# TinfoilHat0/Defending-Against-Backdoors-with-Robust-Learning-Rate

Measured on NVIDIA H100. Metric: fl_rounds_per_sec, higher is better.
Workload: dtype bf16

## Files before the change

### defending-against-backdoors-with-robust-learning-rate_b200/models/native.py

```python
from __future__ import annotations

import math
import os

import torch
import torch.nn.functional as F

from .. import ops
from .graph import FlatLayout

ACT = torch.bfloat16
FUSE_DROPOUT = bool(int(os.environ.get("RLR_FUSE_DROPOUT", "1")))
FUSE_RELU_POOL = bool(int(os.environ.get("RLR_FUSE_RELU_POOL", "1")))
EPILOGUE_BN_STATS = bool(int(os.environ.get("RLR_EPILOGUE_BN_STATS", "0")))
FWD_BRANCH = bool(int(os.environ.get("RLR_FWD_BRANCH", "1")))
BWD_BRANCH = bool(int(os.environ.get("RLR_BWD_BRANCH", "1")))
EPI_STAT_SLOTS = min(16, max(1, int(os.environ.get("RLR_EPI_STAT_SLOTS", "2"))))
FWD_SLOTS = BWD_SLOTS = max(1, int(os.environ.get("RLR_BN_SLOTS", "1")))
WGRAD_OVERLAP = bool(int(os.environ.get("RLR_WGRAD_OVERLAP", "1")))


def dropout_stream_base(seed: int, agent_id: int, rnd: int) -> int:
    z = (int(seed) * 0x9E3779B97F4A7C15 + (int(agent_id) + 1) * 0xBF58476D1CE4E5B9 + (int(rnd) + 1) * 0x94D049BB133111EB) & (2 ** 64 - 1)
    z = ((z ^ (z >> 30)) * 0xBF58476D1CE4E5B9) & (2 ** 64 - 1)
# ... 348 lines not shown
        name = op.name + ".weight"
        gw, gb = self.pg[name], self.pg.get(op.name + ".bias")
        s, p = a.get("stride", 1), a.get("pad", 0)
        if self.impl["conv_wgrad"] == "sm100" and ops.conv_supported(op.in_shape, a, "wgrad"):
            if getattr(self, "_side", None) is not None:
                self._side.wait_stream(torch.cuda.current_stream(self.device))
                with torch.cuda.stream(self._side):
                    ops.conv2d_wgrad_sm100(x, dy, gw, gb, s, p, tag=(id(self), op.name), zero=False)
            else:
                ops.conv2d_wgrad_sm100(x, dy, gw, gb, s, p, tag=(id(self), op.name), zero=False)
        else:
            if self.impl["conv_wgrad"] == "sm100":
                ops.note_fallback("conv_wgrad", f"{op.name} in={op.in_shape} {a}")
            _, dw, db = torch.ops.aten.convolution_backward(
                dy.permute(0, 3, 1, 2), x.permute(0, 3, 1, 2), self.pwb[name].permute(0, 3, 1, 2),
                [a["cout"]] if gb is not None else None, [s, s], [p, p], [1, 1], False, [0, 0], 1, [False, True, gb is not None])
            gw.copy_(dw.permute(0, 2, 3, 1))
            if gb is not None:
                gb.copy_(db)
        if not op.need_dx:
            return
        dx = self.G(op.x, B)
        if self.impl["conv_dgrad"] == "sm100" and ops.conv_supported(op.in_shape, a, "dgrad"):
            ops.conv2d_dgrad_sm100(dy, self.pwb[name], dx, s, p, op.acc_dx)
            return
        if self.impl["conv_dgrad"] == "sm100":
            ops.note_fallback("conv_dgrad", f"{op.name} in={op.in_shape} {a}")
        di, _, _ = torch.ops.aten.convolution_backward(
            dy.permute(0, 3, 1, 2), x.permute(0, 3, 1, 2), self.pwb[name].permute(0, 3, 1, 2), None, [s, s], [p, p], [1, 1],
            False, [0, 0], 1, [True, False, False])
        di = di.permute(0, 2, 3, 1)
        if op.acc_dx:
            dx.add_(di)
        else:
            dx.copy_(di)

    def _fwd_bn(self, op, B, train):
        a = op.attrs
        x, y = self.T(op.x, B), self.T(op.y, B)
        res = self.T(op.res, B) if op.res is not None else None
        gamma, beta = self.pw[op.name + ".weight"], self.pw[op.name + ".bias"]
        rm, rv = self.pw[op.name + ".running_mean"], self.pw[op.name + ".running_var"]
        prod = op.saved["producer"]
        stats = prod.saved["stats"] if (train and prod is not None and prod.saved.get("stats_done")) else None
        if stats is not None and not self.fuse_bn_stats:
            stats = stats[0:EPI_STAT_SLOTS]
        count = x.numel() // x.shape[-1]
# ... 230 lines not shown
```

### defending-against-backdoors-with-robust-learning-rate_b200/ops/__init__.py

```python
from __future__ import annotations

import importlib.util
import os
import threading
from typing import NamedTuple

import numpy as np
import torch

_HERE = os.path.dirname(os.path.abspath(__file__))
_SO = os.path.join(_HERE, "_C.so")
_ext = None
_ext_err = None
_lock = threading.Lock()

MODE_IDS = {"avg": 0, "comed": 1, "sign": 2}
MAX_FUSED_AGENTS = 1024


class _Counter:
    calls = 0


class _CountingExt:
# ... 429 lines not shown
        dl = dl.to(logits.dtype)
        if dlogits is not None:
            dlogits.copy_(dl)
            dl = dlogits
    if loss_sum is None:
        loss_sum = torch.zeros(1)
    loss_sum += loss
    if correct is not None:
        correct += (lf.argmax(1) == labels).sum().to(correct.dtype)
    return loss_sum, dl


def eval_metrics(logits, labels, loss_sum, confusion):
    if logits.is_cuda:
        ext().eval_metrics(logits.contiguous(), labels, loss_sum, confusion)
        return
    lf = logits.float()
    loss_sum += torch.nn.functional.cross_entropy(lf, labels, reduction="sum").double()
    C = lf.shape[1]
    pred = lf.argmax(1)
    confusion.view(-1).index_add_(0, labels * C + pred, torch.ones_like(labels))


from .nn import (avgpool_bwd, avgpool_fwd, bn_bwd, bn_fwd, conv2d_dgrad_sm100, conv2d_fwd_sm100, conv2d_wgrad_sm100, conv_supported,
                 dropout_bwd, dropout_fwd, gn_bwd, gn_fwd, linear_bwd, linear_fused_dropout_ok, linear_fwd, maxpool2_bwd, maxpool2_fwd, relu_bwd_, scratch, stem_geometry, STAT_SLOTS)
```

### defending-against-backdoors-with-robust-learning-rate_b200/ops/csrc/gemm.cu

```cuda
#include <cuda.h>
#include <stdlib.h>

#include "common.cuh"
#include "gemm.h"
#include "stem_gather.cuh"
#include "wgmma.cuh"

namespace rlr {

using namespace wg;

constexpr int BM = 128;
constexpr int BK = 64;
constexpr int kConsumers = 256;
constexpr int kThreads = kConsumers + 64;
constexpr int kEpiThreads = kConsumers;

template <int BN, int kOcc = 2>
struct TileCfg {
    static constexpr int kStages = kOcc == 3 ? (BN == 64 ? 3 : 2) : (BN == 64 ? 4 : 3);
    static constexpr int kABytes = BM * BK * 2;
    static constexpr int kBBytes = BN * BK * 2;
    static constexpr int kStageBytes = kABytes + kBBytes;
    static constexpr int kPitch = BN * 2 + 16;
// ... 445 lines not shown
cudaError_t launch_stem_gemm_bf16(const void* A, const void* W, void* out, int M, int N, int kvalid, int ldw, const float* bias, int relu,
                                  float* stats, const uint32_t* wait_flags, int wait_lo, int wait_hi, const uint32_t* wait_epoch,
                                  cudaStream_t st) {
    if (N % 8 || M <= 0 || kvalid < 1 || kvalid > BK || ldw < kvalid) return cudaErrorInvalidValue;
    if (wait_flags && (!wait_epoch || wait_lo > wait_hi || wait_lo < 0)) return cudaErrorInvalidValue;
    const int m_tiles = (M + BM - 1) / BM;
    const int bn = pick_bn(N);
    CUtensorMap tmA;
    {
        const uint64_t d[2] = {(uint64_t)BK, (uint64_t)M}, s[1] = {(uint64_t)BK * 2};
        const uint32_t b[2] = {BK, BM};
        RLR_CUDA_CHECK(make_tmap_bf16(&tmA, A, 2, d, s, b));
    }
    ConvGemmParams p{};
    p.M = M; p.N = N; p.num_kb = 1; p.mode = 0; p.in_stride = 1; p.out_stride = 1;
    p.out = out; p.ldc = N; p.bias = bias; p.stats = stats; p.relu = relu; p.accumulate = 0;
    p.b_src = reinterpret_cast<const __nv_bfloat16*>(W); p.b_ld = ldw; p.b_kvalid = kvalid;
    p.wait_flags = wait_flags; p.wait_lo = wait_lo; p.wait_hi = wait_hi; p.wait_epoch = wait_epoch;
    return bn == 128 ? launch_bn<128>(tmA, tmA, p, m_tiles, st) : launch_bn<64>(tmA, tmA, p, m_tiles, st);
}

static int pow2_ceil(int x) { int p = 1; while (p < x) p <<= 1; return p; }

cudaError_t launch_conv_bf16(const void* x, const void* w, void* out, int NB, int planes, int Hin, int Win, int Cin, int Ho, int Wo,
                             int Cout, int ldc, int ntaps, const int* dh, const int* dw, const int* dplane, const float* bias,
                             int relu, int accumulate, float* stats, cudaStream_t st, const int* wtap, int w_taps_total,
                             int in_stride, int out_stride, int out_ph, int out_pw) {
    if (Cin % BK || Cout % 8 || ntaps < 1 || ntaps > 9) return cudaErrorInvalidValue;
    if (in_stride < 1 || in_stride > 2 || out_stride < 1 || out_stride > 2 || (in_stride > 1 && planes != 1)) return cudaErrorInvalidValue;
    if (wtap && (stats || Cout % 64)) return cudaErrorInvalidValue;
    int bn = pick_bn(Cout);
    ConvGemmParams p{};
    {
        static const int small_bn64 = [] { const char* e = getenv("RLR_SMALL_BN64"); return e ? atoi(e) : 1; }();
        const long long px = (long long)NB * Ho * Wo;
        if (small_bn64 && bn == 128 && ((px + BM - 1) / BM) * (Cout / 128) < sm_count()) bn = 64;
    }
    int TW = pow2_ceil(Wo); if (TW > BM) TW = BM;
    int TH = pow2_ceil(Ho); if (TW * TH > BM) TH = BM / TW;
    int TN = BM / (TW * TH);
    p.TW = TW; p.TH = TH; p.TN = TN;
    p.tiles_w = (Wo + TW - 1) / TW; p.tiles_h = (Ho + TH - 1) / TH;
    const int tiles_n = (NB + TN - 1) / TN;
    const int m_tiles = p.tiles_w * p.tiles_h * tiles_n;
    p.M = NB * Ho * Wo; p.N = Cout; p.mode = 1; p.cblocks = Cin / BK; p.num_kb = ntaps * p.cblocks; p.ntaps = ntaps;
    p.Ho = Ho; p.Wo = Wo; p.NB = NB;
    p.in_stride = in_stride; p.out_stride = out_stride; p.out_ph = out_ph; p.out_pw = out_pw; p.OutH = Ho * out_stride; p.OutW = Wo * out_stride;
    for (int t = 0; t < ntaps; ++t) { p.dh[t] = (int8_t)dh[t]; p.dw[t] = (int8_t)dw[t]; p.dn[t] = dplane[t] * NB; }
    p.out = out; p.ldc = ldc; p.bias = bias; p.stats = stats; p.relu = relu; p.accumulate = accumulate;
    CUtensorMap tmA, tmB;
    {
        const uint64_t d[4] = {(uint64_t)Cin, (uint64_t)Win, (uint64_t)Hin, (uint64_t)planes * NB};
        const uint64_t s[3] = {(uint64_t)Cin * 2, (uint64_t)Win * Cin * 2, (uint64_t)Hin * Win * Cin * 2};
        const uint32_t b[4] = {BK, (uint32_t)TW, (uint32_t)TH, (uint32_t)TN};
        const uint32_t es[4] = {1, (uint32_t)in_stride, (uint32_t)in_stride, 1};
        RLR_CUDA_CHECK(make_tmap_bf16(&tmA, x, 4, d, s, b, in_stride > 1 ? es : nullptr));
    }
    if (wtap) {
        if (bias) return cudaErrorInvalidValue;
        p.b_mn = 1; p.wcols = Cout;
        for (int t = 0; t < ntaps; ++t) p.wtap[t] = wtap[t];
        const uint64_t cols = (uint64_t)w_taps_total * Cout;
        const uint64_t d[2] = {cols, (uint64_t)Cin}, s[1] = {cols * 2};
        const uint32_t b[2] = {64, BK};
        RLR_CUDA_CHECK(make_tmap_bf16(&tmB, w, 2, d, s, b));
    } else {
        const uint64_t K = (uint64_t)ntaps * Cin;
        const uint64_t d[2] = {K, (uint64_t)Cout}, s[1] = {K * 2};
        const uint32_t b[2] = {BK, (uint32_t)bn};
        RLR_CUDA_CHECK(make_tmap_bf16(&tmB, w, 2, d, s, b));
    }
    return bn == 128 ? launch_bn<128>(tmA, tmB, p, m_tiles, st) : launch_bn<64>(tmA, tmB, p, m_tiles, st);
}

}
```

### defending-against-backdoors-with-robust-learning-rate_b200/ops/csrc/gemm.h

```cpp
#pragma once
#include <cuda_runtime.h>
#include <cuda_bf16.h>
#include <stdint.h>

#include "dropspec.h"

namespace rlr {

constexpr int kStatSlots = 16;

struct ConvGemmParams {
    int M, N, num_kb;
    int mode;
    int cblocks;
    int TW, TH, TN;
    int Ho, Wo, NB;
    int tiles_w, tiles_h;
    int ntaps;
    int in_stride;
    int out_stride, out_ph, out_pw, OutH, OutW;
    int8_t dh[9], dw[9];
    int dn[9];
    int b_mn;
    int wtap[9];
    int wcols;
    DropSpec drop;
    int tma_store;
    int split_prod;
    long long* dbg;
    const __nv_bfloat16* b_src;
    int b_ld, b_kvalid;
    const uint32_t* wait_flags;
    int wait_lo, wait_hi;
    const uint32_t* wait_epoch;
    void* out;
    int ldc;
    const float* bias;
    float* stats;
    int stat_slots;
    int relu, accumulate;
};

cudaError_t launch_gemm_bf16(const void* A, const void* B, void* out, int M, int N, int K, int lda, int ldb, int ldc,
                             const float* bias, int relu, int accumulate, float* stats, cudaStream_t st, const DropSpec* drop = nullptr);
cudaError_t launch_stem_gemm_bf16(const void* A, const void* W, void* out, int M, int N, int kvalid, int ldw, const float* bias, int relu,
                                  float* stats, const uint32_t* wait_flags, int wait_lo, int wait_hi, const uint32_t* wait_epoch,
                                  cudaStream_t st);
void set_pdl(int on);
cudaError_t launch_gemm_splitk_bf16(const void* A, const void* B, void* out, float* ws, int M, int N, int K, const float* bias, int relu,
                                    int num_sms, cudaStream_t st, const DropSpec* drop = nullptr);
void set_persistent_conv(int on);
void set_conv_occ3(int level);
void set_conv_tma_store(int on);
void set_conv_split_producer(int on);
void set_conv_trace(long long* buf);
long long* conv_trace_buf();
cudaError_t launch_conv_bf16(const void* x, const void* w, void* out, int NB, int planes, int Hin, int Win, int Cin, int Ho, int Wo,
                             int Cout, int ldc, int ntaps, const int* dh, const int* dw, const int* dplane, const float* bias,
                             int relu, int accumulate, float* stats, cudaStream_t st, const int* wtap = nullptr, int w_taps_total = 0,
                             int in_stride = 1, int out_stride = 1, int out_ph = 0, int out_pw = 0);

cudaError_t launch_conv3x3_halo_bf16(const void* x, const void* w, void* out, int NB, int Hin, int Win, int H, int W, int Cout, const float* bias,
                                     int relu, int accumulate, float* stats, int bo_mode, long long* dbg, int num_sms, cudaStream_t st);

cudaError_t launch_conv3x3_halo3_bf16(const void* x, const void* w, void* out, int NB, int H, int W, int Cout, const float* bias, int relu,
                                      int accumulate, int num_sms, cudaStream_t st);

cudaError_t launch_conv_wgrad_bf16(const void* dy, const void* x, float* dW, int NB, int planes, int Hin, int Win, int Cin, int Cin_valid,
                                   int Ho, int Wo, int Cout, int ntaps, const int* dh, const int* dw, const int* dplane, int num_sms,
                                   cudaStream_t st, int in_stride = 1);
cudaError_t launch_conv_wgrad_halo_bf16(const void* dy, const void* x, float* dW, int NB, int H, int W, int Cin_valid, int Cout,
                                        int num_sms, cudaStream_t st);
cudaError_t launch_linear_wgrad_bf16(const void* dy, const void* x, float* dW, int B, int N, int K, int num_sms, cudaStream_t st);

cudaError_t launch_ordered_sum_f32(float* out, const float* part, int nparts, long long n, cudaStream_t st);
cudaError_t launch_ordered_sum_f64(double* out, const double* part, int nparts, long long n, cudaStream_t st);
cudaError_t launch_channel_stats(const __nv_bfloat16* x, long long M, int C, float* stats , int num_sms, cudaStream_t st,
                                 int only_sum = 0, int nslots = 1);
cudaError_t launch_bn_finalize(const float* stats, int slots, float* mean_rstd, float* running_mean, float* running_var, int C,
                               float count, float eps, float momentum, int train, cudaStream_t st);
cudaError_t launch_bn_apply(const __nv_bfloat16* x, const __nv_bfloat16* res, __nv_bfloat16* y, const float* gamma, const float* beta,
                            float* mean_rstd, long long M, int C, int relu, int fin_mode, const float* stats, int slots, float count,
                            float eps, float momentum, float* running_mean, float* running_var, int num_sms, cudaStream_t st);
// ... 40 lines not shown
```

### defending-against-backdoors-with-robust-learning-rate_b200/ops/csrc/gemm_binding.cpp

```cpp
#include <torch/extension.h>
#include <ATen/cuda/CUDAContext.h>
#include <c10/cuda/CUDAGuard.h>
#include <c10/cuda/CUDAStream.h>
#include <c10/cuda/CUDACachingAllocator.h>

#include <vector>

#include "gemm.h"

namespace rlr {
void* scratch_alloc(size_t bytes, cudaStream_t st) {
    return c10::cuda::CUDACachingAllocator::raw_alloc_with_stream(bytes < 256 ? 256 : bytes, st);
}
void scratch_free(void* p) { c10::cuda::CUDACachingAllocator::raw_delete(p); }
}

namespace {
inline cudaStream_t cur_stream() { return c10::cuda::getCurrentCUDAStream().stream(); }
inline int num_sms() { return at::cuda::getCurrentDeviceProperties()->multiProcessorCount; }
inline void check(cudaError_t e, const char* what) { TORCH_CHECK(e == cudaSuccess, what, ": ", cudaGetErrorString(e)); }
template <typename T>
inline T* opt(const c10::optional<at::Tensor>& t) { return t.has_value() && t->defined() ? reinterpret_cast<T*>(t->data_ptr()) : nullptr; }
inline const __nv_bfloat16* bf(const at::Tensor& t) {
    TORCH_CHECK(t.is_cuda() && t.scalar_type() == at::kBFloat16 && t.is_contiguous(), "expected contiguous CUDA bf16 tensor");
// ... 64 lines not shown
    const int M = A.size(0), K = A.size(1), N = B.size(0);
    TORCH_CHECK(B.size(1) == K && out.size(0) == M && out.size(1) == N && ws.numel() == (int64_t)M * N);
    check(rlr::launch_gemm_splitk_bf16(bf(A), bf(B), bfm(out), f32(ws), M, N, K, opt<const float>(bias), relu, num_sms(), cur_stream(),
                                       drop.thr ? &drop : nullptr), "gemm_splitk_bf16");
}

void conv_bf16_strided(at::Tensor x, at::Tensor w, at::Tensor out, std::vector<int64_t> dh, std::vector<int64_t> dw,
                       c10::optional<at::Tensor> bias, bool relu, bool accumulate, std::vector<int64_t> wtap, int64_t w_taps_total,
                       int64_t in_stride, int64_t out_stride, int64_t out_ph, int64_t out_pw) {
    c10::cuda::CUDAGuard g(x.device());
    TORCH_CHECK(x.dim() == 4 && out.dim() == 4 && w.dim() == 2 && x.size(0) == out.size(0));
    TORCH_CHECK(out.size(1) % out_stride == 0 && out.size(2) % out_stride == 0, "output image must be a multiple of out_stride");
    const int NB = x.size(0), Hin = x.size(1), Win = x.size(2), Cin = x.size(3), Cout = out.size(3);
    const int Ho = out.size(1) / out_stride, Wo = out.size(2) / out_stride;
    const int T = (int)dh.size();
    const bool bmn = !wtap.empty();
    TORCH_CHECK(bmn ? (w.size(0) == Cin && w.size(1) == w_taps_total * Cout && (int)wtap.size() == T)
                    : (w.size(0) == Cout && w.size(1) == (int64_t)T * Cin), "filter shape");
    int a[9], b[9], c[9] = {0}, wt[9];
    for (int t = 0; t < T; ++t) { a[t] = (int)dh[t]; b[t] = (int)dw[t]; wt[t] = bmn ? (int)wtap[t] : 0; }
    check(rlr::launch_conv_bf16(bf(x), bf(w), bfm(out), NB, 1, Hin, Win, Cin, Ho, Wo, Cout, Cout, T, a, b, c, opt<const float>(bias), relu,
                                accumulate, nullptr, cur_stream(), bmn ? wt : nullptr, (int)w_taps_total, (int)in_stride, (int)out_stride,
                                (int)out_ph, (int)out_pw), "conv_bf16_strided");
}

void conv3x3_halo_bf16(at::Tensor x, at::Tensor w, at::Tensor out, c10::optional<at::Tensor> bias, bool relu, bool accumulate,
                       c10::optional<at::Tensor> stats, int64_t bo_mode, c10::optional<at::Tensor> dbg) {
    c10::cuda::CUDAGuard g(x.device());
    TORCH_CHECK(x.dim() == 4 && x.size(3) == 64 && out.dim() == 4 && w.dim() == 2 && w.size(1) == 9 * 64 && w.size(0) == out.size(3));
    TORCH_CHECK(out.size(0) == x.size(0) && out.size(1) - x.size(1) == out.size(2) - x.size(2), "halo conv: output = input + 2*pad - 2, pad in {0,1,2}");
    TORCH_CHECK(!stats.has_value() || !stats->defined() || stats->numel() == (int64_t)rlr::kStatSlots * 2 * out.size(3), "stats must be [STAT_SLOTS,2,Cout]");
    check(rlr::launch_conv3x3_halo_bf16(bf(x), bf(w), bfm(out), x.size(0), x.size(1), x.size(2), out.size(1), out.size(2), out.size(3), opt<const float>(bias), relu,
                                        accumulate, opt<float>(stats), (int)bo_mode, opt<long long>(dbg), num_sms(), cur_stream()), "conv3x3_halo_bf16");
}

void conv3x3_halo3_bf16(at::Tensor x, at::Tensor w, at::Tensor out, c10::optional<at::Tensor> bias, bool relu, bool accumulate) {
    c10::cuda::CUDAGuard g(x.device());
    TORCH_CHECK(x.dim() == 4 && x.size(3) == 64 && out.dim() == 4 && w.dim() == 2 && w.size(1) == 9 * 64 && w.size(0) == out.size(3));
    TORCH_CHECK(out.size(0) == x.size(0) && out.size(1) == x.size(1) && out.size(2) == x.size(2));
    check(rlr::launch_conv3x3_halo3_bf16(bf(x), bf(w), bfm(out), x.size(0), x.size(1), x.size(2), out.size(3), opt<const float>(bias), relu,
                                         accumulate, num_sms(), cur_stream()), "conv3x3_halo3_bf16");
}

void conv_wgrad_bf16(at::Tensor dy, at::Tensor x, at::Tensor dW, int64_t NB, int64_t planes, int64_t cin_valid, std::vector<int64_t> dh,
                     std::vector<int64_t> dw, std::vector<int64_t> dplane) {
    c10::cuda::CUDAGuard g(x.device());
// ... 216 lines not shown
    check(rlr::launch_linear_small_bwd2(bf(x), bf(dy), bf(w), const_cast<__nv_bfloat16*>(bfo(dx)), (float*)dw.data_ptr(), opt<float>(db),
                                        x.size(0), x.size(1), w.size(0), accumulate_dx, cur_stream()), "linear_small_bwd2");
}
}

void register_gemm_bindings(py::module_& m) {
    m.attr("STAT_SLOTS") = rlr::kStatSlots;
    m.def("set_persistent_conv", [](bool on) { rlr::set_persistent_conv(on ? 1 : 0); });
    m.def("set_pdl", [](bool on) { rlr::set_pdl(on ? 1 : 0); });
    m.def("set_conv_occ3", [](int64_t level) { rlr::set_conv_occ3((int)level); });
    m.def("set_conv_tma_store", [](bool on) { rlr::set_conv_tma_store(on ? 1 : 0); });
    m.def("set_conv_split_producer", [](bool on) { rlr::set_conv_split_producer(on ? 1 : 0); });
    m.def("set_conv_trace", [](c10::optional<at::Tensor> buf) {
        rlr::set_conv_trace(buf.has_value() && buf->defined() ? reinterpret_cast<long long*>(buf->data_ptr<int64_t>()) : nullptr);
    });
    m.def("gemm_bf16", &gemm_bf16, py::arg("A"), py::arg("B"), py::arg("out"), py::arg("bias"), py::arg("relu"), py::arg("accumulate"), py::arg("stats"),
          py::arg("drop_p") = 0.0, py::arg("drop_seed") = 0, py::arg("drop_step") = py::none(), py::arg("drop_stream") = 0);
    m.def("stem_gemm_bf16", &stem_gemm_bf16, py::arg("A"), py::arg("W"), py::arg("out"), py::arg("bias"), py::arg("relu"), py::arg("stats"),
          py::arg("ready_ptr") = 0, py::arg("lo") = 0, py::arg("hi") = 0, py::arg("epoch") = py::none());
    m.def("gemm_splitk_bf16", &gemm_splitk_bf16, py::arg("A"), py::arg("B"), py::arg("out"), py::arg("ws"), py::arg("bias"), py::arg("relu"),
          py::arg("drop_p") = 0.0, py::arg("drop_seed") = 0, py::arg("drop_step") = py::none(), py::arg("drop_stream") = 0);
    m.def("conv_bf16", &conv_bf16);
    m.def("conv_bf16_strided", &conv_bf16_strided);
    m.def("conv_wgrad_bf16_strided", &conv_wgrad_bf16_strided);
    m.def("conv3x3_halo_bf16", &conv3x3_halo_bf16);
    m.def("conv3x3_halo3_bf16", &conv3x3_halo3_bf16);
    m.def("conv_wgrad_bf16", &conv_wgrad_bf16);
    m.def("linear_wgrad_bf16", &linear_wgrad_bf16);
    m.def("conv_wgrad_halo_bf16", &conv_wgrad_halo_bf16);
    m.def("channel_stats", &channel_stats);
    m.def("ordered_sum", &ordered_sum);
    m.def("bias_grad", &bias_grad);
    m.def("bn_finalize", &bn_finalize);
    m.def("bn_apply", &bn_apply);
    m.def("bn_bwd", &bn_bwd);
    m.def("bn_bwd_recompute", &bn_bwd_recompute);
    m.def("gn_fwd", &gn_fwd);
    m.def("gn_bwd", &gn_bwd);
    m.def("relu_bwd", &relu_bwd, py::arg("dy"), py::arg("y"), py::arg("scale") = 1.0);
    m.def("maxpool2_fwd", &maxpool2_fwd, py::arg("x"), py::arg("y"), py::arg("idx"), py::arg("drop_p") = 0.0, py::arg("drop_seed") = 0,
          py::arg("drop_step") = py::none(), py::arg("drop_stream") = 0);
    m.def("maxpool2_bwd", &maxpool2_bwd, py::arg("dy"), py::arg("idx"), py::arg("dx"), py::arg("drop_p") = 0.0, py::arg("drop_seed") = 0,
          py::arg("drop_step") = py::none(), py::arg("drop_stream") = 0, py::arg("relu_out") = py::none());
    m.def("avgpool_fwd", &avgpool_fwd);
    m.def("avgpool_bwd", &avgpool_bwd);
    m.def("dropout_fwd", &dropout_fwd);
// ... 12 lines not shown
```

### defending-against-backdoors-with-robust-learning-rate_b200/ops/csrc/gemm_persistent.cu

```cuda
#include <cuda.h>

#include "common.cuh"
#include "gemm.h"
#include "stem_gather.cuh"
#include "wgmma.cuh"

namespace rlr {

using namespace wg;

constexpr int PBM = 128, PBK = 64, PConsumers = 256, PThreads = PConsumers + 32;

template <int BN, int kOcc = 1>
struct PCfg {
    static constexpr int kStages = kOcc == 2 ? 3 : (BN == 64 ? 7 : 5);
    static constexpr int kABytes = PBM * PBK * 2;
    static constexpr int kBBytes = BN * PBK * 2;
    static constexpr int kStageBytes = kABytes + kBBytes;
    static constexpr int kPitch = BN * 2 + 16;
    static constexpr int kStagingBytes = PBM * kPitch;
    static constexpr int kRingBytes = kStages * kStageBytes;
    static constexpr int kTailBytes = BN == 128 ? 2048 : 1024;
    static constexpr int kSmemBytes = kRingBytes + kStagingBytes + 1024 + kTailBytes;
};
// ... 3 lines not shown
    uint64_t empty[8];
    int row_index[PBM];
};
static_assert(sizeof(PShared) <= 704, "the bias slice starts 704 bytes into the tail");

template <int BN, bool kBMN, int kOcc = 1>
__global__ void __launch_bounds__(PThreads, kOcc)
umma_conv_gemm_persistent_kernel(const __grid_constant__ CUtensorMap tmA, const __grid_constant__ CUtensorMap tmB, const ConvGemmParams p,
                                  const int m_tiles, const int total_tiles) {
    using Cfg = PCfg<BN, kOcc>;
    extern __shared__ uint8_t smem_raw[];
    uint8_t* smem = reinterpret_cast<uint8_t*>((reinterpret_cast<uintptr_t>(smem_raw) + 1023) & ~uintptr_t(1023));
    uint8_t* staging = smem + Cfg::kRingBytes;
    PShared* sh = reinterpret_cast<PShared*>(staging + Cfg::kStagingBytes);
    const int warp = threadIdx.x >> 5, lane = threadIdx.x & 31;

    if (warp == 8 && lane == 0) {
        prefetch_tmap(&tmA); prefetch_tmap(&tmB);
        for (int s = 0; s < Cfg::kStages; ++s) { mbar_init(&sh->full[s], 1); mbar_init(&sh->empty[s], 8); }
        fence_barrier_init();
    }
    __syncthreads();

    auto origin = [&](int tile, int& tile_m, int& tile_n, int& n0, int& h0, int& w0) {
        tile_m = tile % m_tiles; tile_n = tile / m_tiles;
        n0 = h0 = w0 = 0;
        if (p.mode == 1) {
            const int tw_i = tile_m % p.tiles_w, th_i = (tile_m / p.tiles_w) % p.tiles_h, tn_i = tile_m / (p.tiles_w * p.tiles_h);
            w0 = tw_i * p.TW; h0 = th_i * p.TH; n0 = tn_i * p.TN;
        }
    };

    if (warp == 8) {
        if (p.b_src) stem_gather_b(p, smem + Cfg::kABytes, BN, 0, lane);
        if (lane == 0) {
            int stage = 0;
            uint32_t phase = 0;
            for (int tile = blockIdx.x; tile < total_tiles; tile += gridDim.x) {
                int tile_m, tile_n, n0, h0, w0;
                origin(tile, tile_m, tile_n, n0, h0, w0);
                for (int kb = 0; kb < p.num_kb; ++kb) {
                    mbar_wait(&sh->empty[stage], phase ^ 1);
                    uint8_t* sa = smem + stage * Cfg::kStageBytes;
                    uint8_t* sb = sa + Cfg::kABytes;
                    mbar_expect_tx(&sh->full[stage], p.b_src ? Cfg::kABytes : Cfg::kStageBytes);
                    const int tap = p.mode == 1 ? kb / p.cblocks : 0, cb = p.mode == 1 ? kb - tap * p.cblocks : 0;
                    if (p.mode == 1) tma_load_4d(&tmA, &sh->full[stage], sa, cb * PBK, w0 * p.in_stride + p.dw[tap], h0 * p.in_stride + p.dh[tap],
                                                n0 + p.dn[tap]);
                    else tma_load_2d(&tmA, &sh->full[stage], sa, kb * PBK, tile_m * PBM);
                    if (p.b_src) {
                    } else if (kBMN) {
                        for (int g = 0; g < BN / 64; ++g)
                            tma_load_2d(&tmB, &sh->full[stage], sb + g * 8192, p.wtap[tap] * p.wcols + tile_n * BN + g * 64, cb * PBK);
                    } else {
                        tma_load_2d(&tmB, &sh->full[stage], sb, kb * PBK, tile_n * BN);
                    }
                    if (++stage == Cfg::kStages) { stage = 0; phase ^= 1; }
                }
            }
        }
    } else {
        const int et = threadIdx.x;
        const int wgi = et >> 7, t = et & 127;
        const int r0 = wgi * 64 + frag_row(t, 0);
        __nv_bfloat16* out = reinterpret_cast<__nv_bfloat16*>(p.out);
        constexpr int kChunks = BN * 2 / 16;
        constexpr int kIters = PBM * kChunks / PConsumers;
        constexpr int kBatch = kIters < 8 ? kIters : 8;
        float* bias_s = reinterpret_cast<float*>(reinterpret_cast<uint8_t*>(sh) + 704);
        int bias_tile_n = -1;
        int stage = 0;
        uint32_t phase = 0;
        const uint32_t b_fixed = p.b_src ? smem_u32(smem + Cfg::kABytes) : 0u;
        for (int tile = blockIdx.x; tile < total_tiles; tile += gridDim.x) {
            int tile_m, tile_n, n0, h0, w0;
            origin(tile, tile_m, tile_n, n0, h0, w0);
            const int col0 = tile_n * BN;
            if (p.bias && tile_n != bias_tile_n) {
                for (int i = et; i < BN; i += PConsumers) bias_s[i] = (col0 + i < p.N) ? p.bias[col0 + i] : 0.f;
                bias_tile_n = tile_n;
            }
            if (et < PBM) {
                const int row = et;
                int gi;
                if (p.mode == 1) {
                    const int tw = row % p.TW, th = (row / p.TW) % p.TH, tn = row / (p.TW * p.TH);
                    const int w = w0 + tw, h = h0 + th, n = n0 + tn;
                    gi = (w < p.Wo && h < p.Ho && n < p.NB)
                             ? ((n * p.OutH + h * p.out_stride + p.out_ph) * p.OutW + w * p.out_stride + p.out_pw) : -1;
                } else {
                    gi = tile_m * PBM + row;
                    if (gi >= p.M) gi = -1;
                }
                sh->row_index[row] = gi;
            }
            float acc[BN / 2];
#pragma unroll
            for (int i = 0; i < BN / 2; ++i) acc[i] = 0.f;
            consumer_mainloop<BN, Cfg::kStages, Cfg::kStageBytes, Cfg::kABytes, kBMN>(acc, smem, sh->full, sh->empty, p.num_kb,
                                                                                       (uint32_t)wgi * 64 * 128, b_fixed, stage, phase, lane);
            named_bar(1, PConsumers);
#pragma unroll
            for (int j = 0; j < BN / 8; ++j) {
                const int c = frag_col(t, 4 * j);
#pragma unroll
                for (int h = 0; h < 2; ++h) {
                    float a = acc[4 * j + 2 * h], b = acc[4 * j + 2 * h + 1];
                    if (p.bias) { a += bias_s[c]; b += bias_s[c + 1]; }
                    if (p.relu) { a = fmaxf(a, 0.f); b = fmaxf(b, 0.f); }
                    *reinterpret_cast<uint32_t*>(staging + (r0 + 8 * h) * Cfg::kPitch + c * 2) = pack_bf16x2(a, b);
                }
            }
            named_bar(1, PConsumers);
#pragma unroll
            for (int it0 = 0; it0 < kIters; it0 += kBatch) {
                uint4 oldv[kBatch];
                if (p.accumulate) {
#pragma unroll
                    for (int j = 0; j < kBatch; ++j) {
                        const int idx = et + (it0 + j) * PConsumers, r = idx / kChunks, ch = idx - r * kChunks;
                        const int gi = sh->row_index[r];
                        oldv[j] = make_uint4(0, 0, 0, 0);
// ... 7 lines not shown
                    if (gi < 0 || col0 + ch * 8 >= p.N) continue;
                    uint4 val = *reinterpret_cast<const uint4*>(staging + r * Cfg::kPitch + ch * 16);
                    if (p.accumulate) {
                        const __nv_bfloat162* o2 = reinterpret_cast<const __nv_bfloat162*>(&oldv[j]);
                        __nv_bfloat162* v2 = reinterpret_cast<__nv_bfloat162*>(&val);
#pragma unroll
                        for (int q = 0; q < 4; ++q) {
                            const float2 a = __bfloat1622float2(v2[q]), b = __bfloat1622float2(o2[q]);
                            v2[q] = __floats2bfloat162_rn(a.x + b.x, a.y + b.y);
                        }
                    }
                    *reinterpret_cast<uint4*>(out + (size_t)gi * p.ldc + col0 + ch * 8) = val;
                }
            }
            named_bar(1, PConsumers);
        }
    }
}

template <int BN>
cudaError_t launch_persistent_bn(const CUtensorMap& tmA, const CUtensorMap& tmB, const ConvGemmParams& p, int m_tiles, int num_sms,
                                 cudaStream_t st, int occ) {
    const int n_tiles = (p.N + BN - 1) / BN;
    const int total = m_tiles * n_tiles;
    if (occ == 2 && !p.b_mn) {
        using Cfg = PCfg<BN, 2>;
        static bool configured2 = false;
        if (!configured2) {
            RLR_CUDA_CHECK(cudaFuncSetAttribute(umma_conv_gemm_persistent_kernel<BN, false, 2>, cudaFuncAttributeMaxDynamicSharedMemorySize, Cfg::kSmemBytes));
            configured2 = true;
        }
        const int grid = total < 2 * num_sms ? total : 2 * num_sms;
        umma_conv_gemm_persistent_kernel<BN, false, 2><<<grid, PThreads, Cfg::kSmemBytes, st>>>(tmA, tmB, p, m_tiles, total);
        return cudaGetLastError();
    }
    using Cfg = PCfg<BN>;
    static bool configured = false;
    if (!configured) {
        RLR_CUDA_CHECK(cudaFuncSetAttribute(umma_conv_gemm_persistent_kernel<BN, false>, cudaFuncAttributeMaxDynamicSharedMemorySize, Cfg::kSmemBytes));
        RLR_CUDA_CHECK(cudaFuncSetAttribute(umma_conv_gemm_persistent_kernel<BN, true>, cudaFuncAttributeMaxDynamicSharedMemorySize, Cfg::kSmemBytes));
        configured = true;
    }
    const int grid = total < num_sms ? total : num_sms;
    if (p.b_mn) umma_conv_gemm_persistent_kernel<BN, true><<<grid, PThreads, Cfg::kSmemBytes, st>>>(tmA, tmB, p, m_tiles, total);
    else umma_conv_gemm_persistent_kernel<BN, false><<<grid, PThreads, Cfg::kSmemBytes, st>>>(tmA, tmB, p, m_tiles, total);
    return cudaGetLastError();
}
template cudaError_t launch_persistent_bn<64>(const CUtensorMap&, const CUtensorMap&, const ConvGemmParams&, int, int, cudaStream_t, int);
template cudaError_t launch_persistent_bn<128>(const CUtensorMap&, const CUtensorMap&, const ConvGemmParams&, int, int, cudaStream_t, int);

}
```

### defending-against-backdoors-with-robust-learning-rate_b200/ops/nn.py

```python
from __future__ import annotations

import math
import os

import torch
import torch.nn.functional as F

_scratch = {}
_s2d_done = {}
STAT_SLOTS = 16
USE_WGRAD_HALO = True
USE_STRIDED_TMA = bool(int(os.environ.get("RLR_STRIDED_TMA", "1")))
USE_IM2COL_STEM = bool(int(os.environ.get("RLR_IM2COL_STEM", "1")))
USE_BN_RECOMPUTE = bool(int(os.environ.get("RLR_BN_RECOMPUTE", "1")))
USE_HALO3 = bool(int(os.environ.get("RLR_HALO3", "0")))
USE_HALO_ANY = bool(int(os.environ.get("RLR_HALO_ANY", "1")))
USE_SPLITK = bool(int(os.environ.get("RLR_SPLITK", "1")))
USE_HEAD_V2 = bool(int(os.environ.get("RLR_HEAD_V2", "1")))


def _stem_ok(k, stride, cin, cout):
    return USE_IM2COL_STEM and stride == 1 and cin * k * k <= 64 and cout % 8 == 0 and (cout <= 64 or cout % 128 == 0)


# ... 132 lines not shown
    B = dy.shape[0]
    if stride == 2:
        return _conv2d_dgrad_s2(e, dy, w, dx, pad, accumulate)
    if _halo_ok(k, 1, k - 1 - pad, Cout, dy.shape[1], dy.shape[2]) and dx.shape[-1] % 8 == 0:
        wt = scratch(("wt", w.data_ptr(), dx.data_ptr()), (Cin, k * k * Cout), w.dtype, w.device)
        e.filter_transpose(w, wt, Cout, k * k, Cin)
        if USE_HALO3 and pad == 1 and dy.shape[1] % 16 == 0:
            e.conv3x3_halo3_bf16(dy, wt, dx, None, False, bool(accumulate))
        else:
            e.conv3x3_halo_bf16(dy, wt, dx, None, False, bool(accumulate), None, 0, None)
        return dx
    dh, dw, pl = _taps(k, 1, k - 1 - pad)
    if Cin % 64 == 0:
        T = k * k
        e.conv_bf16(dy, w.reshape(Cout, T * Cin), dx, B, 1, dh, dw, pl, None, False, bool(accumulate), None,
                    [T - 1 - t for t in range(T)], T)
        return dx
    wt = scratch(("wt", w.data_ptr(), dx.data_ptr()), (Cin, k * k * Cout), w.dtype, w.device)
    e.filter_transpose(w, wt, Cout, k * k, Cin)
    e.conv_bf16(dy, wt, dx, B, 1, dh, dw, pl, None, False, bool(accumulate), None, [], 0)
    return dx


def _conv2d_dgrad_s2(e, dy, w, dx, pad, accumulate):
    Cout, k, _, Cin = w.shape
    B, Ho, Wo, _ = dy.shape
    plan = []
    for pi in range(2):
        for pj in range(2):
            taps, dh, dw = [], [], []
            for fy in range(k):
                for fx in range(k):
                    if (pi + pad - fy) % 2 == 0 and (pj + pad - fx) % 2 == 0:
                        taps.append(fy * k + fx); dh.append((pi + pad - fy) // 2); dw.append((pj + pad - fx) // 2)
            if taps:
                plan.append((pi, pj, taps, dh, dw))
    if USE_STRIDED_TMA and Cin % 64 == 0 and dx.shape[1] == 2 * Ho and dx.shape[2] == 2 * Wo:
        if not accumulate and len(plan) < 4:
            _zero(dx)
        for pi, pj, taps, dh, dw in plan:
            e.conv_bf16_strided(dy, w.reshape(Cout, k * k * Cin), dx, dh, dw, None, False, bool(accumulate), taps, k * k, 1, 2, pi, pj)
        return dx
    dx4 = scratch(("dx4", w.data_ptr(), dx.data_ptr()), (4 * B, Ho, Wo, Cin), dy.dtype, dy.device)
    mask = 0
    for pi, pj, taps, dh, dw in plan:
        plane = pi * 2 + pj
        mask |= 1 << plane
        if Cin % 64 == 0:
            e.conv_bf16(dy, w.reshape(Cout, k * k * Cin), dx4[plane * B:(plane + 1) * B], B, 1, dh, dw, [0] * len(taps), None,
                        False, False, None, taps, k * k)
            continue
        wt = scratch(("wt_s2", w.data_ptr(), dx.data_ptr(), plane), (Cin, len(taps) * Cout), w.dtype, w.device)
        e.filter_gather_transpose(w, wt, Cout, k * k, Cin, taps)
        e.conv_bf16(dy, wt, dx4[plane * B:(plane + 1) * B], B, 1, dh, dw, [0] * len(taps), None, False, False, None, [], 0)
    e.depth_to_space(dx4, dx, bool(accumulate), mask)
    return dx


def conv2d_wgrad_sm100(x, dy, gw, gb, stride, pad, tag="fwd", zero=True):
# ... 323 lines not shown
```

Measured before the change: 0.6731.

## Group stride-2 dgrad phase planes into one persistent conv kernel launch

Stride-2 3x3 data-gradient convolutions previously launched one strided conv kernel per output phase plane (up to four launches). They now go through a single persistent kernel that indexes tiles across all planes, with a per-plane tap range and output phase offset. Planes are sorted by tap count so the heavier planes are scheduled first. The intent is to cut launch overhead and fill the SMs better on small layers, at the cost of uneven per-tile work and extra per-tile branching in the persistent kernel.

```diff
diff --git a/defending-against-backdoors-with-robust-learning-rate_b200/models/native.py b/defending-against-backdoors-with-robust-learning-rate_b200/models/native.py
--- a/defending-against-backdoors-with-robust-learning-rate_b200/models/native.py
+++ b/defending-against-backdoors-with-robust-learning-rate_b200/models/native.py
@@ -394,7 +394,10 @@
             return
         dx = self.G(op.x, B)
         if self.impl["conv_dgrad"] == "sm100" and ops.conv_supported(op.in_shape, a, "dgrad"):
-            ops.conv2d_dgrad_sm100(dy, self.pwb[name], dx, s, p, op.acc_dx)
+            if s == 2 and dx.is_cuda and ops.dgrad_s2_grouped_ok(self.pwb[name], dy, dx):
+                ops.conv2d_dgrad_s2_grouped_sm100(dy, self.pwb[name], dx, p, op.acc_dx)
+            else:
+                ops.conv2d_dgrad_sm100(dy, self.pwb[name], dx, s, p, op.acc_dx)
             return
         if self.impl["conv_dgrad"] == "sm100":
             ops.note_fallback("conv_dgrad", f"{op.name} in={op.in_shape} {a}")
diff --git a/defending-against-backdoors-with-robust-learning-rate_b200/ops/__init__.py b/defending-against-backdoors-with-robust-learning-rate_b200/ops/__init__.py
--- a/defending-against-backdoors-with-robust-learning-rate_b200/ops/__init__.py
+++ b/defending-against-backdoors-with-robust-learning-rate_b200/ops/__init__.py
@@ -475,5 +475,5 @@
     confusion.view(-1).index_add_(0, labels * C + pred, torch.ones_like(labels))
 
 
-from .nn import (avgpool_bwd, avgpool_fwd, bn_bwd, bn_fwd, conv2d_dgrad_sm100, conv2d_fwd_sm100, conv2d_wgrad_sm100, conv_supported,
-                 dropout_bwd, dropout_fwd, gn_bwd, gn_fwd, linear_bwd, linear_fused_dropout_ok, linear_fwd, maxpool2_bwd, maxpool2_fwd, relu_bwd_, scratch, stem_geometry, STAT_SLOTS)
+from .nn import (avgpool_bwd, avgpool_fwd, bn_bwd, bn_fwd, conv2d_dgrad_s2_grouped_sm100, conv2d_dgrad_sm100, conv2d_fwd_sm100,
+                 conv2d_wgrad_sm100, conv_supported, dgrad_s2_grouped_ok, dropout_bwd, dropout_fwd, gn_bwd, gn_fwd, linear_bwd, linear_fused_dropout_ok, linear_fwd, maxpool2_bwd, maxpool2_fwd, relu_bwd_, scratch, stem_geometry, STAT_SLOTS)
diff --git a/defending-against-backdoors-with-robust-learning-rate_b200/ops/csrc/gemm.cu b/defending-against-backdoors-with-robust-learning-rate_b200/ops/csrc/gemm.cu
--- a/defending-against-backdoors-with-robust-learning-rate_b200/ops/csrc/gemm.cu
+++ b/defending-against-backdoors-with-robust-learning-rate_b200/ops/csrc/gemm.cu
@@ -491,6 +491,23 @@
 
 static int pow2_ceil(int x) { int p = 1; while (p < x) p <<= 1; return p; }
 
+static int conv_pick_bn(int Cout, long long px) {
+    int bn = pick_bn(Cout);
+    static const int small_bn64 = [] { const char* e = getenv("RLR_SMALL_BN64"); return e ? atoi(e) : 1; }();
+    if (small_bn64 && bn == 128 && ((px + BM - 1) / BM) * (Cout / 128) < sm_count()) bn = 64;
+    return bn;
+}
+
+static int conv_tiling(ConvGemmParams& p, int NB, int Ho, int Wo) {
+    int TW = pow2_ceil(Wo); if (TW > BM) TW = BM;
+    int TH = pow2_ceil(Ho); if (TW * TH > BM) TH = BM / TW;
+    int TN = BM / (TW * TH);
+    p.TW = TW; p.TH = TH; p.TN = TN;
+    p.tiles_w = (Wo + TW - 1) / TW; p.tiles_h = (Ho + TH - 1) / TH;
+    const int tiles_n = (NB + TN - 1) / TN;
+    return p.tiles_w * p.tiles_h * tiles_n;
+}
+
 cudaError_t launch_conv_bf16(const void* x, const void* w, void* out, int NB, int planes, int Hin, int Win, int Cin, int Ho, int Wo,
                              int Cout, int ldc, int ntaps, const int* dh, const int* dw, const int* dplane, const float* bias,
                              int relu, int accumulate, float* stats, cudaStream_t st, const int* wtap, int w_taps_total,
@@ -498,20 +515,10 @@
     if (Cin % BK || Cout % 8 || ntaps < 1 || ntaps > 9) return cudaErrorInvalidValue;
     if (in_stride < 1 || in_stride > 2 || out_stride < 1 || out_stride > 2 || (in_stride > 1 && planes != 1)) return cudaErrorInvalidValue;
     if (wtap && (stats || Cout % 64)) return cudaErrorInvalidValue;
-    int bn = pick_bn(Cout);
+    const int bn = conv_pick_bn(Cout, (long long)NB * Ho * Wo);
     ConvGemmParams p{};
-    {
-        static const int small_bn64 = [] { const char* e = getenv("RLR_SMALL_BN64"); return e ? atoi(e) : 1; }();
-        const long long px = (long long)NB * Ho * Wo;
-        if (small_bn64 && bn == 128 && ((px + BM - 1) / BM) * (Cout / 128) < sm_count()) bn = 64;
-    }
-    int TW = pow2_ceil(Wo); if (TW > BM) TW = BM;
-    int TH = pow2_ceil(Ho); if (TW * TH > BM) TH = BM / TW;
-    int TN = BM / (TW * TH);
-    p.TW = TW; p.TH = TH; p.TN = TN;
-    p.tiles_w = (Wo + TW - 1) / TW; p.tiles_h = (Ho + TH - 1) / TH;
-    const int tiles_n = (NB + TN - 1) / TN;
-    const int m_tiles = p.tiles_w * p.tiles_h * tiles_n;
+    const int m_tiles = conv_tiling(p, NB, Ho, Wo);
+    const int TW = p.TW, TH = p.TH, TN = p.TN;
     p.M = NB * Ho * Wo; p.N = Cout; p.mode = 1; p.cblocks = Cin / BK; p.num_kb = ntaps * p.cblocks; p.ntaps = ntaps;
     p.Ho = Ho; p.Wo = Wo; p.NB = NB;
     p.in_stride = in_stride; p.out_stride = out_stride; p.out_ph = out_ph; p.out_pw = out_pw; p.OutH = Ho * out_stride; p.OutW = Wo * out_stride;
@@ -542,4 +549,47 @@
     return bn == 128 ? launch_bn<128>(tmA, tmB, p, m_tiles, st) : launch_bn<64>(tmA, tmB, p, m_tiles, st);
 }
 
-}
+constexpr int kDgradS2Occ = 2;
+
+cudaError_t launch_conv_dgrad_s2_grouped_bf16(const void* dy, const void* w, void* out, int NB, int Ho, int Wo, int Cin, int Cout,
+                                              int ntaps, const int* dh, const int* dw, const int* wtap, int w_taps_total, int nplanes,
+                                              const int* plane_t0, const int* plane_nt, const int* plane_ph, const int* plane_pw,
+                                              int accumulate, int num_sms, cudaStream_t st) {
+    if (Cin % BK || Cout % 64 || ntaps < 1 || ntaps > 9 || nplanes < 1 || nplanes > 4 || w_taps_total < 1) return cudaErrorInvalidValue;
+    ConvGemmParams p{};
+    p.nplanes = nplanes;
+    for (int i = 0; i < nplanes; ++i) {
+        if (plane_t0[i] < 0 || plane_nt[i] < 1 || plane_t0[i] + plane_nt[i] > ntaps || (plane_ph[i] & ~1) || (plane_pw[i] & ~1))
+            return cudaErrorInvalidValue;
+        p.plane_t0[i] = (int8_t)plane_t0[i]; p.plane_nt[i] = (int8_t)plane_nt[i];
+        p.plane_ph[i] = (int8_t)plane_ph[i]; p.plane_pw[i] = (int8_t)plane_pw[i];
+    }
+    for (int t = 0; t < ntaps; ++t) {
+        if (wtap[t] < 0 || wtap[t] >= w_taps_total) return cudaErrorInvalidValue;
+        p.dh[t] = (int8_t)dh[t]; p.dw[t] = (int8_t)dw[t]; p.dn[t] = 0; p.wtap[t] = wtap[t];
+    }
+    const int bn = conv_pick_bn(Cout, (long long)NB * Ho * Wo);
+    const int m_tiles = conv_tiling(p, NB, Ho, Wo);
+    p.M = NB * Ho * Wo; p.N = Cout; p.mode = 1; p.cblocks = Cin / BK; p.num_kb = 0; p.ntaps = ntaps;
+    p.Ho = Ho; p.Wo = Wo; p.NB = NB;
+    p.in_stride = 1; p.out_stride = 2; p.OutH = 2 * Ho; p.OutW = 2 * Wo;
+    p.b_mn = 1; p.wcols = Cout;
+    p.out = out; p.ldc = Cout; p.accumulate = accumulate;
+    CUtensorMap tmA, tmB;
+    {
+        const uint64_t d[4] = {(uint64_t)Cin, (uint64_t)Wo, (uint64_t)Ho, (uint64_t)NB};
+        const uint64_t s[3] = {(uint64_t)Cin * 2, (uint64_t)Wo * Cin * 2, (uint64_t)Ho * Wo * Cin * 2};
+        const uint32_t b[4] = {BK, (uint32_t)p.TW, (uint32_t)p.TH, (uint32_t)p.TN};
+        RLR_CUDA_CHECK(make_tmap_bf16(&tmA, dy, 4, d, s, b));
+    }
+    {
+        const uint64_t cols = (uint64_t)w_taps_total * Cout;
+        const uint64_t d[2] = {cols, (uint64_t)Cin}, s[1] = {cols * 2};
+        const uint32_t b[2] = {64, BK};
+        RLR_CUDA_CHECK(make_tmap_bf16(&tmB, w, 2, d, s, b));
+    }
+    return bn == 128 ? launch_persistent_bn<128>(tmA, tmB, p, m_tiles, num_sms, st, 1)
+                     : launch_persistent_bn<64>(tmA, tmB, p, m_tiles, num_sms, st, kDgradS2Occ);
+}
+
+}
diff --git a/defending-against-backdoors-with-robust-learning-rate_b200/ops/csrc/gemm.h b/defending-against-backdoors-with-robust-learning-rate_b200/ops/csrc/gemm.h
--- a/defending-against-backdoors-with-robust-learning-rate_b200/ops/csrc/gemm.h
+++ b/defending-against-backdoors-with-robust-learning-rate_b200/ops/csrc/gemm.h
@@ -24,6 +24,8 @@
     int b_mn;
     int wtap[9];
     int wcols;
+    int nplanes;
+    int8_t plane_t0[4], plane_nt[4], plane_ph[4], plane_pw[4];
     DropSpec drop;
     int tma_store;
     int split_prod;
@@ -59,6 +61,10 @@
                              int Cout, int ldc, int ntaps, const int* dh, const int* dw, const int* dplane, const float* bias,
                              int relu, int accumulate, float* stats, cudaStream_t st, const int* wtap = nullptr, int w_taps_total = 0,
                              int in_stride = 1, int out_stride = 1, int out_ph = 0, int out_pw = 0);
+cudaError_t launch_conv_dgrad_s2_grouped_bf16(const void* dy, const void* w, void* out, int NB, int Ho, int Wo, int Cin, int Cout,
+                                              int ntaps, const int* dh, const int* dw, const int* wtap, int w_taps_total, int nplanes,
+                                              const int* plane_t0, const int* plane_nt, const int* plane_ph, const int* plane_pw,
+                                              int accumulate, int num_sms, cudaStream_t st);
 
 cudaError_t launch_conv3x3_halo_bf16(const void* x, const void* w, void* out, int NB, int Hin, int Win, int H, int W, int Cout, const float* bias,
                                      int relu, int accumulate, float* stats, int bo_mode, long long* dbg, int num_sms, cudaStream_t st);
diff --git a/defending-against-backdoors-with-robust-learning-rate_b200/ops/csrc/gemm_binding.cpp b/defending-against-backdoors-with-robust-learning-rate_b200/ops/csrc/gemm_binding.cpp
--- a/defending-against-backdoors-with-robust-learning-rate_b200/ops/csrc/gemm_binding.cpp
+++ b/defending-against-backdoors-with-robust-learning-rate_b200/ops/csrc/gemm_binding.cpp
@@ -110,6 +110,25 @@
     check(rlr::launch_conv_bf16(bf(x), bf(w), bfm(out), NB, 1, Hin, Win, Cin, Ho, Wo, Cout, Cout, T, a, b, c, opt<const float>(bias), relu,
                                 accumulate, nullptr, cur_stream(), bmn ? wt : nullptr, (int)w_taps_total, (int)in_stride, (int)out_stride,
                                 (int)out_ph, (int)out_pw), "conv_bf16_strided");
+}
+
+void conv_dgrad_s2_grouped_bf16(at::Tensor dy, at::Tensor w, at::Tensor out, std::vector<int64_t> dh, std::vector<int64_t> dw,
+                                std::vector<int64_t> wtap, int64_t w_taps_total, std::vector<int64_t> plane_t0, std::vector<int64_t> plane_nt,
+                                std::vector<int64_t> plane_ph, std::vector<int64_t> plane_pw, bool accumulate) {
+    c10::cuda::CUDAGuard g(dy.device());
+    TORCH_CHECK(dy.dim() == 4 && out.dim() == 4 && w.dim() == 2 && dy.size(0) == out.size(0), "conv_dgrad_s2_grouped: shapes");
+    TORCH_CHECK(out.size(1) == 2 * dy.size(1) && out.size(2) == 2 * dy.size(2), "conv_dgrad_s2_grouped: dX must be exactly 2x dY");
+    const int NB = dy.size(0), Ho = dy.size(1), Wo = dy.size(2), Cin = dy.size(3), Cout = out.size(3);
+    const int T = (int)dh.size(), P = (int)plane_t0.size();
+    TORCH_CHECK(T >= 1 && T <= 9 && (int)dw.size() == T && (int)wtap.size() == T, "conv_dgrad_s2_grouped: 1..9 taps");
+    TORCH_CHECK(P >= 1 && P <= 4 && (int)plane_nt.size() == P && (int)plane_ph.size() == P && (int)plane_pw.size() == P,
+                "conv_dgrad_s2_grouped: 1..4 planes");
+    TORCH_CHECK(w.size(0) == Cin && w.size(1) == w_taps_total * Cout, "filter shape");
+    int a[9], b[9], wt[9], t0[4], nt[4], ph[4], pw[4];
+    for (int t = 0; t < T; ++t) { a[t] = (int)dh[t]; b[t] = (int)dw[t]; wt[t] = (int)wtap[t]; }
+    for (int i = 0; i < P; ++i) { t0[i] = (int)plane_t0[i]; nt[i] = (int)plane_nt[i]; ph[i] = (int)plane_ph[i]; pw[i] = (int)plane_pw[i]; }
+    check(rlr::launch_conv_dgrad_s2_grouped_bf16(bf(dy), bf(w), bfm(out), NB, Ho, Wo, Cin, Cout, T, a, b, wt, (int)w_taps_total, P, t0, nt,
+                                                 ph, pw, accumulate, num_sms(), cur_stream()), "conv_dgrad_s2_grouped_bf16");
 }
 
 void conv3x3_halo_bf16(at::Tensor x, at::Tensor w, at::Tensor out, c10::optional<at::Tensor> bias, bool relu, bool accumulate,
@@ -372,6 +391,7 @@
           py::arg("drop_p") = 0.0, py::arg("drop_seed") = 0, py::arg("drop_step") = py::none(), py::arg("drop_stream") = 0);
     m.def("conv_bf16", &conv_bf16);
     m.def("conv_bf16_strided", &conv_bf16_strided);
+    m.def("conv_dgrad_s2_grouped_bf16", &conv_dgrad_s2_grouped_bf16);
     m.def("conv_wgrad_bf16_strided", &conv_wgrad_bf16_strided);
     m.def("conv3x3_halo_bf16", &conv3x3_halo_bf16);
     m.def("conv3x3_halo3_bf16", &conv3x3_halo3_bf16);
diff --git a/defending-against-backdoors-with-robust-learning-rate_b200/ops/csrc/gemm_persistent.cu b/defending-against-backdoors-with-robust-learning-rate_b200/ops/csrc/gemm_persistent.cu
--- a/defending-against-backdoors-with-robust-learning-rate_b200/ops/csrc/gemm_persistent.cu
+++ b/defending-against-backdoors-with-robust-learning-rate_b200/ops/csrc/gemm_persistent.cu
@@ -49,7 +49,15 @@
     }
     __syncthreads();
 
-    auto origin = [&](int tile, int& tile_m, int& tile_n, int& n0, int& h0, int& w0) {
+    auto origin = [&](int tile, int& tile_m, int& tile_n, int& n0, int& h0, int& w0, int& t0, int& num_kb, int& ph, int& pw) {
+        t0 = 0; num_kb = p.num_kb; ph = p.out_ph; pw = p.out_pw;
+        if (p.nplanes) {
+            const int per_plane = total_tiles / p.nplanes, pl = tile / per_plane;
+            tile -= pl * per_plane;
+#pragma unroll
+            for (int i = 0; i < 4; ++i)
+                if (i == pl) { t0 = p.plane_t0[i]; num_kb = p.plane_nt[i] * p.cblocks; ph = p.plane_ph[i]; pw = p.plane_pw[i]; }
+        }
         tile_m = tile % m_tiles; tile_n = tile / m_tiles;
         n0 = h0 = w0 = 0;
         if (p.mode == 1) {
@@ -64,14 +72,14 @@
             int stage = 0;
             uint32_t phase = 0;
             for (int tile = blockIdx.x; tile < total_tiles; tile += gridDim.x) {
-                int tile_m, tile_n, n0, h0, w0;
-                origin(tile, tile_m, tile_n, n0, h0, w0);
-                for (int kb = 0; kb < p.num_kb; ++kb) {
+                int tile_m, tile_n, n0, h0, w0, t0, num_kb, ph, pw;
+                origin(tile, tile_m, tile_n, n0, h0, w0, t0, num_kb, ph, pw);
+                for (int kb = 0; kb < num_kb; ++kb) {
                     mbar_wait(&sh->empty[stage], phase ^ 1);
                     uint8_t* sa = smem + stage * Cfg::kStageBytes;
                     uint8_t* sb = sa + Cfg::kABytes;
                     mbar_expect_tx(&sh->full[stage], p.b_src ? Cfg::kABytes : Cfg::kStageBytes);
-                    const int tap = p.mode == 1 ? kb / p.cblocks : 0, cb = p.mode == 1 ? kb - tap * p.cblocks : 0;
+                    const int kt = p.mode == 1 ? kb / p.cblocks : 0, cb = p.mode == 1 ? kb - kt * p.cblocks : 0, tap = t0 + kt;
                     if (p.mode == 1) tma_load_4d(&tmA, &sh->full[stage], sa, cb * PBK, w0 * p.in_stride + p.dw[tap], h0 * p.in_stride + p.dh[tap],
                                                 n0 + p.dn[tap]);
                     else tma_load_2d(&tmA, &sh->full[stage], sa, kb * PBK, tile_m * PBM);
@@ -100,8 +108,8 @@
         uint32_t phase = 0;
         const uint32_t b_fixed = p.b_src ? smem_u32(smem + Cfg::kABytes) : 0u;
         for (int tile = blockIdx.x; tile < total_tiles; tile += gridDim.x) {
-            int tile_m, tile_n, n0, h0, w0;
-            origin(tile, tile_m, tile_n, n0, h0, w0);
+            int tile_m, tile_n, n0, h0, w0, t0, num_kb, ph, pw;
+            origin(tile, tile_m, tile_n, n0, h0, w0, t0, num_kb, ph, pw);
             const int col0 = tile_n * BN;
             if (p.bias && tile_n != bias_tile_n) {
                 for (int i = et; i < BN; i += PConsumers) bias_s[i] = (col0 + i < p.N) ? p.bias[col0 + i] : 0.f;
@@ -114,7 +122,7 @@
                     const int tw = row % p.TW, th = (row / p.TW) % p.TH, tn = row / (p.TW * p.TH);
                     const int w = w0 + tw, h = h0 + th, n = n0 + tn;
                     gi = (w < p.Wo && h < p.Ho && n < p.NB)
-                             ? ((n * p.OutH + h * p.out_stride + p.out_ph) * p.OutW + w * p.out_stride + p.out_pw) : -1;
+                             ? ((n * p.OutH + h * p.out_stride + ph) * p.OutW + w * p.out_stride + pw) : -1;
                 } else {
                     gi = tile_m * PBM + row;
                     if (gi >= p.M) gi = -1;
@@ -124,7 +132,7 @@
             float acc[BN / 2];
 #pragma unroll
             for (int i = 0; i < BN / 2; ++i) acc[i] = 0.f;
-            consumer_mainloop<BN, Cfg::kStages, Cfg::kStageBytes, Cfg::kABytes, kBMN>(acc, smem, sh->full, sh->empty, p.num_kb,
+            consumer_mainloop<BN, Cfg::kStages, Cfg::kStageBytes, Cfg::kABytes, kBMN>(acc, smem, sh->full, sh->empty, num_kb,
                                                                                        (uint32_t)wgi * 64 * 128, b_fixed, stage, phase, lane);
             named_bar(1, PConsumers);
 #pragma unroll
@@ -178,15 +186,23 @@
 cudaError_t launch_persistent_bn(const CUtensorMap& tmA, const CUtensorMap& tmB, const ConvGemmParams& p, int m_tiles, int num_sms,
                                  cudaStream_t st, int occ) {
     const int n_tiles = (p.N + BN - 1) / BN;
-    const int total = m_tiles * n_tiles;
-    if (occ == 2 && !p.b_mn) {
+    const int total = m_tiles * n_tiles * (p.nplanes ? p.nplanes : 1);
+    if (occ == 2) {
+        if (BN != 64 && p.b_mn) return cudaErrorInvalidValue;
         using Cfg = PCfg<BN, 2>;
         static bool configured2 = false;
         if (!configured2) {
             RLR_CUDA_CHECK(cudaFuncSetAttribute(umma_conv_gemm_persistent_kernel<BN, false, 2>, cudaFuncAttributeMaxDynamicSharedMemorySize, Cfg::kSmemBytes));
+            if constexpr (BN == 64)
+                RLR_CUDA_CHECK(cudaFuncSetAttribute(umma_conv_gemm_persistent_kernel<BN, true, 2>, cudaFuncAttributeMaxDynamicSharedMemorySize, Cfg::kSmemBytes));
             configured2 = true;
         }
         const int grid = total < 2 * num_sms ? total : 2 * num_sms;
+        if constexpr (BN == 64)
+            if (p.b_mn) {
+                umma_conv_gemm_persistent_kernel<BN, true, 2><<<grid, PThreads, Cfg::kSmemBytes, st>>>(tmA, tmB, p, m_tiles, total);
+                return cudaGetLastError();
+            }
         umma_conv_gemm_persistent_kernel<BN, false, 2><<<grid, PThreads, Cfg::kSmemBytes, st>>>(tmA, tmB, p, m_tiles, total);
         return cudaGetLastError();
     }
diff --git a/defending-against-backdoors-with-robust-learning-rate_b200/ops/nn.py b/defending-against-backdoors-with-robust-learning-rate_b200/ops/nn.py
--- a/defending-against-backdoors-with-robust-learning-rate_b200/ops/nn.py
+++ b/defending-against-backdoors-with-robust-learning-rate_b200/ops/nn.py
@@ -178,9 +178,7 @@
     return dx
 
 
-def _conv2d_dgrad_s2(e, dy, w, dx, pad, accumulate):
-    Cout, k, _, Cin = w.shape
-    B, Ho, Wo, _ = dy.shape
+def _dgrad_s2_plan(k, pad):
     plan = []
     for pi in range(2):
         for pj in range(2):
@@ -191,6 +189,38 @@
                         taps.append(fy * k + fx); dh.append((pi + pad - fy) // 2); dw.append((pj + pad - fx) // 2)
             if taps:
                 plan.append((pi, pj, taps, dh, dw))
+    return plan
+
+
+def dgrad_s2_grouped_ok(w, dy, dx):
+    _, k, _, Cin = w.shape
+    return (USE_STRIDED_TMA and k == 3 and Cin % 64 == 0 and dx.shape[1] == 2 * dy.shape[1] and dx.shape[2] == 2 * dy.shape[2])
+
+
+def dgrad_s2_grouped_table(k, pad):
+    plan = sorted(_dgrad_s2_plan(k, pad), key=lambda pl: -len(pl[2]))
+    dh, dw, taps, t0, nt, ph, pw = [], [], [], [], [], [], []
+    for pi, pj, ptaps, pdh, pdw in plan:
+        t0.append(len(taps)); nt.append(len(ptaps)); ph.append(pi); pw.append(pj)
+        dh += pdh; dw += pdw; taps += ptaps
+    return dh, dw, taps, t0, nt, ph, pw
+
+
+def conv2d_dgrad_s2_grouped_sm100(dy, w, dx, pad, accumulate):
+    assert dgrad_s2_grouped_ok(w, dy, dx), "grouped stride-2 data gradient: 3x3, Cin % 64 == 0, dX exactly 2x dY"
+    e = _ext()
+    Cout, k, _, Cin = w.shape
+    dh, dw, taps, t0, nt, ph, pw = dgrad_s2_grouped_table(k, pad)
+    if not accumulate and len(t0) < 4:
+        _zero(dx)
+    e.conv_dgrad_s2_grouped_bf16(dy, w.reshape(Cout, k * k * Cin), dx, dh, dw, taps, k * k, t0, nt, ph, pw, bool(accumulate))
+    return dx
+
+
+def _conv2d_dgrad_s2(e, dy, w, dx, pad, accumulate):
+    Cout, k, _, Cin = w.shape
+    B, Ho, Wo, _ = dy.shape
+    plan = _dgrad_s2_plan(k, pad)
     if USE_STRIDED_TMA and Cin % 64 == 0 and dx.shape[1] == 2 * Ho and dx.shape[2] == 2 * Wo:
         if not accumulate and len(plan) < 4:
             _zero(dx)
```

Result: faster. 0.6819, median of 6 (+1.3%).
